# ziqin-h/GIVEPose

Measured on AMD Instinct MI355X. Metric: images/sec PoseNet fwd, bs=64 256x256 fp16, 1/2/4/8 MI355X; % MFMA roofline, higher is better.
Workload: dtype f16

## Files before the change

### givepose_amd/_lib.py

```python
import ctypes
import os
from ctypes import POINTER, Structure, c_char_p, c_double, c_float, c_int, c_long, c_void_p

_HERE = os.path.dirname(os.path.abspath(__file__))
LIB_PATH = os.environ.get("GP_LIB_PATH") or os.path.join(_HERE, "libgivepose_hip.so")

ABI_VERSION = 326
GP_F32, GP_F16, GP_F64 = 0, 1, 2
ACT_NONE, ACT_GELU, ACT_RELU, ACT_LRELU = 0, 1, 2, 3
EPI_NONE, EPI_GELU, EPI_RELU, EPI_LRELU, EPI_SCALE_RES, EPI_RES_RELU, EPI_LNFOLD_GELU = 0, 1, 2, 3, 4, 5, 6
ROT_6D, ROT_6D_Y, ROT_6D_Z, ROT_QUAT, ROT_EULER = 0, 1, 2, 3, 4
KC_GEMM, KC_DCNV3, KC_DWCONV_LN, KC_NORM, KC_ELEMENTWISE, KC_SMALL, KC_COUNT = 0, 1, 2, 3, 4, 5, 6
KC_NAMES = ["gemm", "dcnv3", "dwconv_ln", "norm", "elementwise", "small"]


class GemmDesc(Structure):
    _fields_ = [("X", c_void_p), ("W", c_void_p), ("bias", c_void_p), ("gamma", c_void_p), ("residual", c_void_p),
                ("C", c_void_p), ("workspace", c_void_p),
                ("M", c_int), ("N", c_int), ("K", c_int), ("ldx", c_int), ("ldc", c_int), ("ldres", c_int),
                ("epilogue", c_int), ("out_f32", c_int), ("splitk", c_int),
                ("B", c_int), ("H", c_int), ("Win", c_int), ("Cin", c_int), ("KH", c_int), ("KW", c_int),
                ("stride", c_int), ("pad", c_int), ("Ho", c_int), ("Wo", c_int), ("dtype", c_int),
                ("gn_partial", c_void_p), ("gn_groups", c_int), ("gn_hw", c_int), ("variant", c_int),
                ("ln_stats", c_void_p), ("ln_colsum", c_void_p), ("ln_nslab", c_int), ("ln_eps", c_float),
                ("co_scheduled", c_int), ("prefetch", c_void_p), ("prefetch_bytes", c_long),
                ("split_shift", c_int), ("x_plane_stride", c_long), ("w_plane_stride", c_long),
                ("out_planes", c_int), ("c_plane_stride", c_long),
                ("residual_f32", c_int), ("c16", c_void_p), ("ldc16", c_int), ("gn_rows", c_int)]


# ... 5 lines not shown
    "gp_dcnv3_forward": ([_P, _P, _P, _P] + [c_int] * 9 + [c_float] + [c_int] * 7 + [_P], c_int),
    "gp_dcnv3_forward_any": ([_P] * 4 + [c_int] * 13 + [c_float] + [c_int] * 3 + [_P], c_int),
    "gp_dcnv3_backward": ([_P] * 7 + [c_long, c_long] + [c_int] * 13 + [c_float] + [c_int] * 3 + [_P], c_int),
    "gp_gemm": ([POINTER(GemmDesc), _P], c_int),
    "gp_gemm_gn_rows": ([c_int] * 4, c_int),
    "gp_split_planes": ([_P, _P, c_long, c_int, c_long, c_long, c_int, _P], c_int),
    "gp_convnext_mlp_pack_w2": ([_P, _P, c_int, _P], c_int),
    "gp_convnext_mlp_pack_w2_s32": ([_P, _P, c_int, _P], c_int),
    "gp_convnext_mlp": ([_P] * 8 + [c_long, c_int, c_int, _P], c_int),
    "gp_convnext_stem": ([_P] * 6 + [c_int] * 4 + [c_float, c_int, _P], c_int),
    "gp_dwconv_ln": ([_P] * 6 + [c_int] * 5 + [c_float, c_int, c_long, c_int, _P], c_int),
    "gp_dwconv_ln_groups": ([_P] * 6 + [c_int] * 5 + [c_float, c_int, _P, c_int, _P], c_int),
    "gp_dwconv7_raw_stats": ([_P] * 5 + [c_int] * 5 + [_P], c_int),
    "gp_layernorm": ([_P] * 4 + [c_long, c_int, c_float, c_int, c_int, _P], c_int),
    "gp_groupnorm_chunks": ([c_int, c_int], c_int),
    "gp_groupnorm_stats": ([_P] * 2 + [c_int] * 5 + [_P], c_int),
    "gp_groupnorm_apply": ([_P] * 5 + [c_int] * 4 + [c_float] + [c_int] * 4 + [_P], c_int),
    "gp_groupnorm_upsample2x": ([_P] * 5 + [c_int] * 5 + [c_float] + [c_int] * 3 + [_P], c_int),
    "gp_groupnorm_apply_xyz": ([_P] * 8 + [c_int] * 4 + [c_float] + [c_int] * 3 + [_P], c_int),
    "gp_upsample_bilinear2x": ([_P, _P] + [c_int] * 5 + [_P], c_int),
    "gp_deconv_col2im": ([_P, _P] + [c_int] * 5 + [_P], c_int),
    "gp_xyz_out_layer": ([_P] * 5 + [c_int] * 4 + [_P], c_int),
    "gp_pointwise_k3": ([_P] * 4 + [c_long, c_int, c_int, _P], c_int),
    "gp_pnp_conv1": ([_P] * 4 + [c_int] * 4 + [_P], c_int),
    "gp_xyz_conv3x3_s2": ([_P] * 3 + [c_int] * 4 + [_P], c_int),
    "gp_size_head": ([_P] * 8 + [c_int] * 5 + [_P], c_int),
    "gp_pose_tail": ([_P, _P, c_int] + [_P] * 10 + [c_int, c_int] + [_P] * 5 + [c_int, _P], c_int),
    "gp_pose_tail_rt": ([_P, _P, c_int] + [_P] * 10 + [c_int] * 5 + [_P] * 5 + [c_int, _P], c_int),
    "gp_pnp_conv1_masked": ([_P] * 5 + [c_int] * 4 + [_P], c_int),
    "gp_pool_mmm": ([_P, _P] + [c_int] * 5 + [_P], c_int),
    "gp_patchify_xyz": ([_P, _P, c_int, c_int, c_int, c_int, _P], c_int),
    "gp_attention64": ([_P, _P, c_int, c_int, c_int, _P], c_int),
    "gp_attention64_hd": ([_P, _P] + [c_int] * 4 + [_P], c_int),
    "gp_patchify_pnp": ([_P, _P, _P] + [c_int] * 4 + [_P], c_int),
    "gp_resnet_stem": ([_P] * 4 + [c_int] * 4 + [_P], c_int),
    "gp_maxpool3x3s2": ([_P, _P] + [c_int] * 5 + [_P], c_int),
    "gp_mask_resize_nearest": ([_P, _P, c_int, c_int, c_int, _P], c_int),
    "gp_crop_rois": ([_P] * 12 + [c_int] * 7 + [_P], c_int),
    "gp_pred_rt": ([_P] * 6 + [c_int, _P], c_int),
    "gp_pack_poses": ([_P] * 4 + [c_int, _P], c_int),
    "gp_sn_stem": ([_P] * 4 + [c_int] * 3 + [_P], c_int),
    "gp_sn_pointwise": ([_P] * 6 + [c_long] + [c_int] * 4 + [_P], c_int),
    "gp_sn_depthwise": ([_P] * 4 + [c_int] * 7 + [_P], c_int),
    "gp_sn_avgpool": ([_P] * 2 + [c_int] * 3 + [_P], c_int),
    "gp_sn_se": ([_P] * 6 + [c_int] * 3 + [_P], c_int),
    "gp_sn_head": ([_P] * 12 + [c_int] * 5 + [_P], c_int),
# ... 53 lines not shown
```

### givepose_amd/csrc/dcnv3.hip

```cpp
#include "common.hpp"

namespace {

struct DcnKP {
    const void* in;
    const void* off;
    const void* mask;
    void* out;
    int N, H, W, G, D, K, stride, pad, dil, rc, Ho, Wo, off_ld, mask_ld, logits, xcd;
    float os;
    long rows;
};

template <typename T> struct Ch4;
template <> struct Ch4<half_t> {
    half4 v;
    __device__ __forceinline__ float get(int i) const { return (float)v[i]; }
    __device__ __forceinline__ float fma(float a, int i, float c) const { return fmaf(a, (float)v[i], c); }
    __device__ __forceinline__ float mul(float a, int i) const { return a * (float)v[i]; }
};
template <> struct Ch4<float> {
    f32x4 v;
    __device__ __forceinline__ float get(int i) const { return v[i]; }
    __device__ __forceinline__ float mul(float a, int i) const { return a * v[i]; }
// ... 394 lines not shown

template <typename T, typename OT> int launch(const DcnKP& p, hipStream_t s) {
    if constexpr (sizeof(T) == 2) {
        if (p.G == 4 && p.D == 64 && p.K == 3 && !p.rc && p.Ho % 4 == 0 && p.Wo % 4 == 0 && dcn_patch_enabled() && dcn_wave8_enabled() && !dcn_fold_enabled()) {
            if (dcn_ldsbc_enabled()) hipLaunchKernelGGL((dcnv3_wave8_kernel<OT, true>), dim3(p.N * (p.Ho / 4) * (p.Wo / 4), 2), dim3(256), 0, s, p);
            else hipLaunchKernelGGL((dcnv3_wave8_kernel<OT, false>), dim3(p.N * (p.Ho / 4) * (p.Wo / 4), 2), dim3(256), 0, s, p);
            return 0;
        }
    }
    if (p.G == 4 && p.D == 64 && p.K == 3 && !p.rc && p.Ho % 4 == 0 && p.Wo % 4 == 0 && dcn_patch_enabled()) {
        if (sizeof(T) == 2 && dcn_fold_enabled()) hipLaunchKernelGGL((dcnv3_wave_kernel<T, OT, 3, true, true>), dim3(p.N * (p.Ho / 4) * (p.Wo / 4), 4), dim3(256), 0, s, p);
        else hipLaunchKernelGGL((dcnv3_wave_kernel<T, OT, 3, true>), dim3(p.N * (p.Ho / 4) * (p.Wo / 4), 4), dim3(256), dcn_lds_pad(), s, p);
    } else if (p.G == 4 && p.D == 64 && p.K == 3 && !p.rc) {
        hipLaunchKernelGGL((dcnv3_wave_kernel<T, OT, 3>), dim3(cdiv(p.rows, 4)), dim3(256), 0, s, p);
    } else if (p.G == 4 && p.D == 64 && p.K * p.K - p.rc <= 16) {
        hipLaunchKernelGGL((dcnv3_wave_kernel<T, OT>), dim3(cdiv(p.rows, 4)), dim3(256), 0, s, p);
    } else {
        const long total = p.rows * p.G * (p.D / 4);
        hipLaunchKernelGGL((dcnv3_generic_kernel<T, OT>), dim3(cdiv(total, 256)), dim3(256), 0, s, p);
    }
    return 0;
}

}

extern "C" int gp_dcnv3_forward(const void* in, const void* offset, const void* mask, void* out, int N, int H,
                                int W, int G, int D, int K, int stride, int pad, int dil, float offset_scale,
                                int remove_center, int im2col_step, int off_ld, int mask_ld,
                                int mask_is_logits, int dtype, int om_dtype, void* stream) {
    GP_REQUIRE(in && offset && mask && out, "gp_dcnv3_forward: null pointer");
    GP_REQUIRE(N > 0 && H > 0 && W > 0 && G > 0 && D > 0 && K > 0 && stride > 0 && dil > 0 && pad >= 0,
               "gp_dcnv3_forward: bad geometry");
    GP_REQUIRE(D % 4 == 0, "gp_dcnv3_forward: group_channels=%d must be a multiple of 4", D);
    GP_REQUIRE((dtype == GP_F32 || dtype == GP_F16) && (om_dtype == GP_F32 || om_dtype == GP_F16),
               "gp_dcnv3_forward: bad dtype");
    GP_REQUIRE(!remove_center || (K % 2 == 1), "remove_center is only compatible with odd kernel size.");
    const int step = im2col_step < N ? im2col_step : N;
    GP_REQUIRE(step > 0 && N % step == 0, "batch(%d) must divide im2col_step(%d)", N, step);
    DcnKP p;
    p.in = in; p.off = offset; p.mask = mask; p.out = out;
    p.N = N; p.H = H; p.W = W; p.G = G; p.D = D; p.K = K; p.stride = stride; p.pad = pad; p.dil = dil;
    p.rc = remove_center ? 1 : 0;
    p.Ho = (H + 2 * pad - (dil * (K - 1) + 1)) / stride + 1;
    p.Wo = (W + 2 * pad - (dil * (K - 1) + 1)) / stride + 1;
    GP_REQUIRE(p.Ho > 0 && p.Wo > 0, "gp_dcnv3_forward: empty output");
    const int P = K * K - p.rc;
// ... 16 lines not shown
```

### givepose_amd/csrc/misc.hip

```cpp
#include "common.hpp"

namespace {

__device__ __forceinline__ void store_T(half_t* p, float v) { *p = (half_t)v; }
__device__ __forceinline__ void store_T(float* p, float v) { *p = v; }

template <typename T>
__global__ __launch_bounds__(256) void stem_kernel(const float* __restrict__ img, const float* __restrict__ wt,
                                                   const float* __restrict__ bias, const float* __restrict__ lnw,
                                                   const float* __restrict__ lnb, T* __restrict__ out, int H,
                                                   int W, float eps, int PXB) {
    constexpr int C0 = 128;
    __shared__ __attribute__((aligned(16))) float in_s[12][256];
    const int Ho = H / 4, Wo = W / 4;
    const int tid = threadIdx.x, lane = tid & 63, wave = tid >> 6;
    const int nwb = Wo / PXB;
    const int wblk = blockIdx.x % nwb;
    const int ho = (blockIdx.x / nwb) % Ho;
    const int b = blockIdx.x / (nwb * Ho);
    const int wo0 = wblk * PXB;
    for (int i = tid; i < 12 * PXB * 4; i += 256) {
        const int row = i / (PXB * 4), col = i - row * (PXB * 4);
        const int c = row >> 2, kh = row & 3;
        in_s[row][col] = img[(((long)b * 3 + c) * H + (ho * 4 + kh)) * W + wo0 * 4 + col];
// ... 1037 lines not shown
    GP_REQUIRE(x && w && b && out_nchw && out_nhwc4 && B > 0, "gp_xyz_out_layer: bad argument");
    GP_DT_OK(dtype);
    const int esz = dtype == GP_F16 ? 2 : 4, vec = 16 / esz, chunks = C / vec;
    GP_REQUIRE(C % vec == 0 && (chunks & (chunks - 1)) == 0, "gp_xyz_out_layer: C=%d", C);
    const int LPP = chunks < 64 ? chunks : 64, ppw = 64 / LPP;
    const long rows = (long)B * HW;
    hipStream_t s = (hipStream_t)stream;
    gp_timing_before(s, GP_KC_SMALL, 6.0 * rows * C, (double)rows * C * esz + rows * 28.0);
    dim3 grid(cdiv(rows, 4L * ppw));
    if (dtype == GP_F16) hipLaunchKernelGGL(xyz_out_kernel<half_t>, grid, dim3(256), 0, s, (const half_t*)x, w, b, out_nchw, out_nhwc4, rows, HW, C);
    else hipLaunchKernelGGL(xyz_out_kernel<float>, grid, dim3(256), 0, s, (const float*)x, w, b, out_nchw, out_nhwc4, rows, HW, C);
    GP_LAUNCH_CHECK("gp_xyz_out_layer");
}

extern "C" int gp_pointwise_k3(const float* xyz4, const float* w, const float* b, void* y, long rows, int Cout,
                               int dtype, void* stream) {
    GP_REQUIRE(xyz4 && w && b && y && rows > 0, "gp_pointwise_k3: bad argument");
    GP_DT_OK(dtype);
    const int esz = dtype == GP_F16 ? 2 : 4, vec = 16 / esz;
    GP_REQUIRE(Cout % vec == 0 && 256 % (Cout / vec) == 0, "gp_pointwise_k3: Cout=%d", Cout);
    hipStream_t s = (hipStream_t)stream;
    const long total = cdiv(rows, (256 / (Cout / vec)) * 8) * 256;
    gp_timing_before(s, GP_KC_ELEMENTWISE, 6.0 * rows * Cout, rows * 16.0 + (double)rows * Cout * esz);
    if (dtype == GP_F16) hipLaunchKernelGGL(pointwise_k3_kernel<half_t>, dim3(cdiv(total, 256)), dim3(256), 0, s, xyz4, w, b, (half_t*)y, rows, Cout);
    else hipLaunchKernelGGL(pointwise_k3_kernel<float>, dim3(cdiv(total, 256)), dim3(256), 0, s, xyz4, w, b, (float*)y, rows, Cout);
    GP_LAUNCH_CHECK("gp_pointwise_k3");
}

template <int CIN>
static int launch_smallcin(const float* xyz4, const float* coord2d, const float* w, void* y, int B, int R, int Cout,
                           int dtype, void* stream, const char* name, const float* mask = nullptr) {
    GP_REQUIRE(xyz4 && w && y && B > 0 && R % 8 == 0, "%s: bad argument", name);
    GP_DT_OK(dtype);
    GP_REQUIRE(Cout % 4 == 0 && Cout / 4 <= 256 && 256 % (Cout / 4) == 0, "%s: Cout=%d", name, Cout);
    hipStream_t s = (hipStream_t)stream;
    const long pix = (long)B * (R / 2) * (R / 2);
        const size_t lds = (size_t)CIN * 9 * Cout * sizeof(float);
    gp_timing_before(s, GP_KC_SMALL, 2.0 * pix * CIN * 9 * Cout, (double)B * R * R * CIN * 4 + (double)pix * Cout * (dtype == GP_F16 ? 2 : 4));
    static const bool mfma = [] { const char* e = getenv("GP_SMALLCIN_MFMA"); return !(e && e[0] == '0'); }();
    if (dtype == GP_F16 && mfma && R == 64 && (Cout == 128 || Cout == 256)) {
        if (Cout == 128) hipLaunchKernelGGL((smallcin_conv3x3s2_mfma_kernel<CIN, 2>), dim3(B * (R / 4)), dim3(256), 0, s, xyz4, coord2d, w, (half_t*)y, B, R, mask);
        else hipLaunchKernelGGL((smallcin_conv3x3s2_mfma_kernel<CIN, 4>), dim3(B * (R / 4)), dim3(256), 0, s, xyz4, coord2d, w, (half_t*)y, B, R, mask);
    } else if (dtype == GP_F16)
        hipLaunchKernelGGL((smallcin_conv3x3s2_kernel<half_t, CIN>), dim3(cdiv(pix / 4, 256 / (Cout / 4))), dim3(256), lds, s, xyz4, coord2d, w, (half_t*)y, B, R, Cout, mask);
    else
        hipLaunchKernelGGL((smallcin_conv3x3s2_kernel<float, CIN>), dim3(cdiv(pix / 4, 256 / (Cout / 4))), dim3(256), lds, s, xyz4, coord2d, w, (float*)y, B, R, Cout, mask);
// ... 220 lines not shown
```

### givepose_amd/ops.py

```python
import ctypes
import os

import torch

from . import _lib
from ._lib import (ACT_GELU, ACT_LRELU, ACT_NONE, ACT_RELU, EPI_GELU, EPI_LNFOLD_GELU, EPI_LRELU, EPI_NONE, EPI_RELU, EPI_RES_RELU,
                   EPI_SCALE_RES, GP_F16, GP_F32, GP_F64, GemmDesc, check)

__all__ = ["dtype_code", "gemm", "conv2d_nhwc", "dcnv3_forward", "dcnv3_backward", "dcnv3_forward_into", "convnext_stem", "dwconv_ln",
           "layernorm", "groupnorm", "upsample_bilinear2x", "deconv_col2im", "xyz_out_layer", "pointwise_k3",
           "pnp_conv1", "pnp_conv1_masked", "pool_mmm", "xyz_conv3x3_s2", "size_head", "pose_tail", "pose_tail_rt", "mask_resize_nearest"]


def _L():
    return _lib.load()


def _stream():
    return ctypes.c_void_p(torch.cuda.current_stream().cuda_stream)


def dtype_code(dt):
    if dt == torch.float16:
        return GP_F16
    if dt == torch.float32:
        return GP_F32
    raise TypeError(f"unsupported dtype {dt} (float16 / float32)")


def _ptr(t):
    return None if t is None else ctypes.c_void_p(t.data_ptr())

# ... 421 lines not shown
          "gp_upsample_bilinear2x")
    return out


def deconv_col2im(cols, out, B, H, W_, C):
    code = dtype_code(out.dtype) | (0x400 if cols.dtype == torch.float16 else 0)
    check(_L().gp_deconv_col2im(_ptr(cols), _ptr(out), B, H, W_, C, code, _stream()), "gp_deconv_col2im")
    return out


def xyz_out_layer(x, w, b, out_nchw, out_nhwc4):
    B, HW, C = x.shape
    check(_L().gp_xyz_out_layer(_ptr(_contig(x, "x")), _ptr(w), _ptr(b), _ptr(out_nchw), _ptr(out_nhwc4), B, HW, C,
                                dtype_code(x.dtype), _stream()), "gp_xyz_out_layer")


def pointwise_k3(xyz4, w, b, out):
    rows = xyz4.shape[0]
    check(_L().gp_pointwise_k3(_ptr(xyz4), _ptr(w), _ptr(b), _ptr(out), rows, w.shape[0], dtype_code(out.dtype), _stream()),
          "gp_pointwise_k3")
    return out


def pnp_conv1(xyz4, coord2d, w, out, B, R):
    check(_L().gp_pnp_conv1(_ptr(xyz4), _ptr(_contig(coord2d, "coord2d")), _ptr(w), _ptr(out), B, R, w.shape[1],
                            dtype_code(out.dtype), _stream()), "gp_pnp_conv1")
    return out


def pnp_conv1_masked(xyz4, coord2d, mask, w, out, B, R):
    check(_L().gp_pnp_conv1_masked(_ptr(xyz4), _ptr(_contig(coord2d, "coord2d")), _ptr(_contig(_chk(mask, "mask", torch.float32), "mask")),
                                   _ptr(w), _ptr(out), B, R, w.shape[1], dtype_code(out.dtype), _stream()), "gp_pnp_conv1_masked")
    return out


def pool_mmm(x, out, k):
    B, HW, C = x.shape
    if x.dtype != out.dtype or tuple(out.shape) != (B, k * C):
        raise ValueError(f"pool_mmm: out {tuple(out.shape)} {out.dtype} for x {tuple(x.shape)} {x.dtype}, k={k}")
    check(_L().gp_pool_mmm(_ptr(_contig(x, "x")), _ptr(_contig(out, "out")), B, HW, C, k, dtype_code(x.dtype), _stream()), "gp_pool_mmm")
    return out


def xyz_conv3x3_s2(xyz4, w, out, B, R):
    check(_L().gp_xyz_conv3x3_s2(_ptr(xyz4), _ptr(w), _ptr(out), B, R, w.shape[1], dtype_code(out.dtype), _stream()),
          "gp_xyz_conv3x3_s2")
# ... 47 lines not shown
```

### givepose_amd/posenet.py

```python
import ctypes
import os
from collections import OrderedDict

import numpy as np
import torch
import torch.nn as nn

from . import _lib, ops, synth
from ._lib import (ACT_GELU, ACT_RELU, EPI_GELU, EPI_LNFOLD_GELU, EPI_LRELU, EPI_NONE, EPI_SCALE_RES)
from .config import FLAT_OPS, ROT_TYPES, PoseNetConfig, validate

OM_LD = 128


class _Node(nn.Module):
    """Container mirroring one level of the reference module tree (names only)."""


def _register(root, name, tensor, is_param):
    parts = name.split(".")
    mod = root
    for p in parts[:-1]:
        if p not in mod._modules:
            mod.add_module(p, _Node())
        mod = mod._modules[p]
    if is_param:
        mod.register_parameter(parts[-1], tensor)
    else:
        mod.register_buffer(parts[-1], tensor)


FUSE_GN_UPSAMPLE = os.environ.get("GP_FUSE_GN_UPSAMPLE", "1") != "0"

_BUFFER_SUFFIXES = ("running_mean", "running_var", "num_batches_tracked")

# ... 145 lines not shown
                W[q + "qkv_w"] = gw(a(f"block.{i}.attn.qkv.weight"))
                W[q + "proj_w"], W[q + "proj_b"] = gw(a(f"block.{i}.attn.proj.weight")), f32(a(f"block.{i}.attn.proj.bias"))
                W[q + "fc1_w"], W[q + "fc1_b"] = gw(a(f"block.{i}.mlp.fc1.weight")), f32(a(f"block.{i}.mlp.fc1.bias"))
                W[q + "fc2_w"], W[q + "fc2_b"] = gw(a(f"block.{i}.mlp.fc2.weight")), f32(a(f"block.{i}.mlp.fc2.bias"))
        for li, i in enumerate((0, 3, 6) if cfg.nocsmap_encoder == "conv" else ()):
            p, q = f"nocs_encoder.features.{i}.", f"enc{li}."
            if cfg.use_dcn == "dcnv3":
                cw = sd[p + "conv.weight"].reshape(256, -1)
                W[q + "conv_w"] = f32(cw) if li == 0 else gw(cw)
                W[q + "conv_b"] = f32(sd[p + "conv.bias"])
                d = p + "dcnv3."
                W[q + "dw_w"] = lowp(sd[d + "dw_conv.0.weight"].reshape(256, 9).t())
                W[q + "dw_b"] = f32(sd[d + "dw_conv.0.bias"])
                W[q + "ln_w"], W[q + "ln_b"] = f32(sd[d + "dw_conv.1.1.weight"]), f32(sd[d + "dw_conv.1.1.bias"])
                omw = torch.cat([sd[d + "offset.weight"], sd[d + "mask.weight"]], 0)
                omb = torch.cat([sd[d + "offset.bias"], sd[d + "mask.bias"]], 0)
                W[q + "om_w"] = gw(torch.cat([omw, omw.new_zeros(OM_LD - omw.shape[0], omw.shape[1])], 0))
                W[q + "om_b"] = f32(torch.cat([omb, omb.new_zeros(OM_LD - omb.shape[0])], 0))
                W[q + "in_w"], W[q + "in_b"] = gw(sd[d + "input_proj.weight"]), f32(sd[d + "input_proj.bias"])
                wf = sd[d + "input_proj.weight"] @ cw
                W[q + "fold_w"] = f32(wf) if li == 0 else gw(wf)
                W[q + "fold_b"] = f32(sd[d + "input_proj.weight"] @ sd[p + "conv.bias"] + sd[d + "input_proj.bias"])
                W[q + "out_w"], W[q + "out_b"] = gw(sd[d + "output_proj.weight"]), f32(sd[d + "output_proj.bias"])
            else:
                cw = sd[p + "weight"]
                W[q + "conv_w"] = f32(cw.reshape(256, -1).t()) if li == 0 else gw(cw.permute(0, 2, 3, 1).reshape(256, -1))
            W[q + "gn_w"], W[q + "gn_b"] = f32(sd[f"nocs_encoder.features.{i + 1}.weight"]), f32(sd[f"nocs_encoder.features.{i + 1}.bias"])
        W["red.w"], W["red.b"] = gw(sd["feat_reducer.weight"].reshape(256, -1)), f32(sd["feat_reducer.bias"])
        if cfg.pnp_head == "att":
            a = lambda k: sd["pnp_net." + k]
            W["apn.pe_w"] = gw(a("patch_embed.proj.weight").permute(0, 2, 3, 1).reshape(192, -1))
            W["apn.pe_b"] = f32(a("patch_embed.proj.bias"))
            W["apn.pos"] = f32(a("pos_embed").reshape(64, 192))
            W["apn.ones"] = torch.ones(192, dtype=torch.float32, device=device)
            W["apn.norm_w"], W["apn.norm_b"] = f32(a("norm.weight")), f32(a("norm.bias"))
            for i in range(3):
                q = f"apn{i}."
                for n in ("norm1", "norm2"):
                    W[q + n + "_w"], W[q + n + "_b"] = f32(a(f"block.{i}.{n}.weight")), f32(a(f"block.{i}.{n}.bias"))
                W[q + "qkv_w"] = gw(a(f"block.{i}.attn.qkv.weight"))
                W[q + "proj_w"], W[q + "proj_b"] = gw(a(f"block.{i}.attn.proj.weight")), f32(a(f"block.{i}.attn.proj.bias"))
                W[q + "fc1_w"], W[q + "fc1_b"] = gw(a(f"block.{i}.mlp.fc1.weight")), f32(a(f"block.{i}.mlp.fc1.bias"))
                W[q + "fc2_w"], W[q + "fc2_b"] = gw(a(f"block.{i}.mlp.fc2.weight")), f32(a(f"block.{i}.mlp.fc2.bias"))
        else:
            W["pnp.c0_w"] = f32(sd["pnp_net.features.0.weight"].reshape(128, -1).t())
            for li, i in enumerate((0, 3, 6)):
# ... 53 lines not shown
                h = S // (2 << li)
                for n in ("a", "b", "c"):
                    buf[f"rs{li}{n}"] = e(B, h, h, planes)
        for s, d in enumerate(dims):
            h = H >> s
            if cfg.res_fp32 and T == torch.float16 and d == 512:
                buf[f"x{s}"], buf[f"x{s}h"] = f(B, h, h, d), e(B, h, h, d)
            else:
                buf[f"x{s}"] = e(B, h, h, d)
            buf[f"t{s}"] = e(B, h, h, d)
            buf[f"h{s}"] = e(B * h * h, 4 * d)
            if d == 512:
                buf["ln_stats"] = f(B * h * h, 2, d // 128)
            if s > 0:
                buf[f"dsn{s}"] = e(B, h * 2, h * 2, dims[s - 1])
        buf["cols"] = e(B * 64, 9 * 256) if (T == torch.float16 and cfg.deconv_cols_f16 and os.environ.get("GP_DECONV_COLS_F32") != "1") else f(B * 64, 9 * 256)
        for r in (16, 32, 64):
            buf[f"ya{r}"], buf[f"yb{r}"] = e(B, r, r, 256), e(B, r, r, 256)
        chunks = max(ops.groupnorm_chunks(B, r * r) for r in (8, 16, 32, 64))
        buf["gn_partial"], buf["size_scratch"] = f(B * max(chunks, R * R // 16) * 32 * 2), f(B * (cfg.feat_ts + (512 if cfg.main_backbone == "resnet34" else cfg.convnext_dims[-1])))
        buf["nocs_nchw"], buf["nocs_nhwc4"] = f(B, 3, R, R), f(B * R * R, 4)
        buf["ivfc_nchw"], buf["ivfc_nhwc4"] = f(B, 3, R, R), f(B * R * R, 4)
        buf["mask_out"], buf["size"] = f(B, 1, R, R), f(B, 3)
        for li, r in enumerate((64, 32, 16)):
            buf[f"e_in{li}"], buf[f"e_proj{li}"] = e(B, r, r, 256), e(B, r, r, 256)
            buf[f"e_x1{li}"] = e(B * r * r // 4, 256)
            buf[f"e_om{li}"] = f(B * r * r // 4, OM_LD)
            buf[f"e_g{li}"], buf[f"e_o{li}"] = e(B, r // 2, r // 2, 256), e(B, r // 2, r // 2, 256)
        if cfg.nocsmap_encoder == "att":
            buf["a_patch"], buf["a_x"], buf["a_h"] = e(B * 64, 192), e(B * 64, 256), e(B * 64, 256)
            buf["a_qkv"], buf["a_att"], buf["a_mlp"] = e(B * 64, 768), e(B * 64, 256), e(B * 64, 1024)
            buf["a_pos"] = self._packed["att.pos"].to(T).repeat(B, 1).contiguous()
        buf["feat_cat"] = e(B, 8, 8, 512)
        if cfg.pnp_head == "att":
            buf["p_patch"], buf["p_x"], buf["p_h"] = e(B * 64, 320), e(B * 64, 192), e(B * 64, 192)
            buf["p_qkv"], buf["p_att"], buf["p_mlp"], buf["p_flat"] = e(B * 64, 576), e(B * 64, 192), e(B * 64, 768), e(B * 64, 192)
            buf["p_pos"] = self._packed["apn.pos"].to(T).repeat(B, 1).contiguous()
        else:
            buf["p0"], buf["p1"], buf["p2"] = e(B, 32, 32, 128), e(B, 16, 16, 128), e(B, 8, 8, 128)
        buf["fc1"] = e(B, 2048)
        buf["hh"], buf["hz"] = f(B, 256), f(B, 256)
        if FLAT_OPS[cfg.flat_op]:
            buf["pooled"] = e(B, 128 * FLAT_OPS[cfg.flat_op])
        buf["pred_rot"], buf["pred_t"], buf["rot_allo"], buf["rot_ego"], buf["trans"] = f(B, cfg.rot_dim), f(B, 3), f(B, 9), f(B, 9), f(B, 3)
        buf["rot6d"] = buf["pred_rot"] if cfg.rot_dim == 6 else None
        plan = {"buf": buf, "graph": None, "warm": False, "ragged": bool(ragged)}
        if ragged:
            buf["grp"] = torch.arange(B, dtype=torch.int32, device=device)
            buf["grp_host"] = torch.arange(B, dtype=torch.int32).pin_memory()
            for k in ("roi_img", "roi_mask", "roi_coord_2d", "bbox_center", "mean_size"):
                buf[k].zero_()
            buf["roi_wh"].fill_(1.0)
            buf["resize_ratio"].fill_(1.0)
            buf["cam_K"].copy_(torch.eye(3, device=device).expand(B, 3, 3))
        self._plans[key] = plan
        self._evict_plans(key)
        return plan

    def _gn(self, x, w, b, act, buf, G=32, out=None, ldy=None, fused=False, out_planes=False, rows=64):
        B = x.shape[0]
        C = x.shape[-1]
        xv = x.view(B, -1, C)
        ops.groupnorm(xv, w, b, xv if out is None else out, G, act, buf["gn_partial"], ldy=ldy, fused_stats=fused, out_planes=out_planes, rows=rows)

    def _gnrows(self, M, N, K, hw):
        if self.split_gemm or self.compute_dtype != torch.float16 or os.environ.get("GP_GN_ROWS64") == "1":
            return 64
        return ops.gemm_gn_rows(M, N, K, hw)

# ... 126 lines not shown
            ops.gemm(buf["a_patch"], W["att.pe_w"], x, bias=W["att.pe_b"], epilogue=EPI_SCALE_RES, gamma=W["att.ones"],
                     residual=buf["a_pos"])
            for i in range(3):
                q = f"att{i}."
                h = ops.layernorm(x, W[q + "norm1_w"], W[q + "norm1_b"], buf["a_h"], eps=1e-5)
                ops.gemm(h, W[q + "qkv_w"], buf["a_qkv"])
                ops.attention64(buf["a_qkv"], buf["a_att"], B, 8)
                ops.gemm(buf["a_att"], W[q + "proj_w"], x, bias=W[q + "proj_b"], epilogue=EPI_SCALE_RES, gamma=W["att.ones"], residual=x)
                h = ops.layernorm(x, W[q + "norm2_w"], W[q + "norm2_b"], buf["a_h"], eps=1e-5)
                ops.gemm(h, W[q + "fc1_w"], buf["a_mlp"], bias=W[q + "fc1_b"], epilogue=EPI_GELU)
                ops.gemm(buf["a_mlp"], W[q + "fc2_w"], x, bias=W[q + "fc2_b"], epilogue=EPI_SCALE_RES, gamma=W["att.ones"], residual=x)
            ops.layernorm(x, W["att.norm_w"], W["att.norm_b"], cat2d[:, 256:], eps=1e-5, ldy=512)
        for li, r in enumerate((64, 32, 16) if cfg.nocsmap_encoder == "conv" else ()):
            q = f"enc{li}."
            ro = r // 2
            if only_layer is not None:
                if li != only_layer:
                    continue
                prev = buf[f"e_o{li - 1}"]
                if weights_of is not None:
                    q = f"enc{weights_of}."
            if cfg.use_dcn == "dcnv3":
                xin = buf[f"e_in{li}"]
                if li == 0:
                    ops.pointwise_k3(buf["nocs_nhwc4"], W[q + "fold_w"], W[q + "fold_b"], buf[f"e_proj{li}"].view(-1, 256))
                else:
                    ops.gemm(prev.view(-1, 256), W[q + "fold_w"], buf[f"e_proj{li}"].view(-1, 256), bias=W[q + "fold_b"])
                if plan.get("ragged"):
                    if li == 0:
                        ops.pointwise_k3(buf["nocs_nhwc4"], W[q + "conv_w"], W[q + "conv_b"], xin.view(-1, 256))
                    else:
                        ops.gemm(prev.view(-1, 256), W[q + "conv_w"], xin.view(-1, 256), bias=W[q + "conv_b"])
                    ops.dwconv_ln_groups(xin, W[q + "dw_w"], W[q + "dw_b"], W[q + "ln_w"], W[q + "ln_b"], buf[f"e_x1{li}"], 3, buf["grp"], act=ACT_GELU)
                    ops.gemm(buf[f"e_x1{li}"], W[q + "om_w"], buf[f"e_om{li}"], bias=W[q + "om_b"])
                    ops.dcnv3_forward_into(buf[f"e_proj{li}"], buf[f"e_om{li}"], buf[f"e_om{li}"][:, 72:], buf[f"e_g{li}"], 3, 2, 1, 1, 4, 64, 1.0,
                                           off_ld=OM_LD, mask_ld=OM_LD, mask_is_logits=True)
                Bg = self.dcn_couple if (self.dcn_couple and B > self.dcn_couple) else B
                if plan.get("ragged"):
                    Bg = B + 1
                if B % Bg and not plan.get("ragged"):
                    raise ValueError(f"batch {B} is not a multiple of dcn_couple = {Bg}")
                for g0 in range(0, B if not plan.get("ragged") else 0, Bg):
                    gs = slice(g0, g0 + Bg)
                    nq = Bg * ro * ro
                    npre = min(Bg * r * r, (nq + r + 8 + 15) // 16 * 16)
                    xin_g = xin[gs]
                    if li == 0:
                        ops.pointwise_k3(buf["nocs_nhwc4"][g0 * r * r:][:npre], W[q + "conv_w"], W[q + "conv_b"], xin_g.view(-1, 256)[:npre])
                    else:
                        ops.gemm(prev[gs].view(-1, 256)[:npre], W[q + "conv_w"], xin_g.view(-1, 256)[:npre], bias=W[q + "conv_b"])
                    x1_g = buf[f"e_x1{li}"][g0 * r * r // 4:(g0 + Bg) * r * r // 4]
                    om_g = buf[f"e_om{li}"][g0 * r * r // 4:(g0 + Bg) * r * r // 4]
                    ops.dwconv_ln(xin_g, W[q + "dw_w"], W[q + "dw_b"], W[q + "ln_w"], W[q + "ln_b"], x1_g, 3, act=ACT_GELU, n_pixels=nq)
                    ops.gemm(x1_g, W[q + "om_w"], om_g, bias=W[q + "om_b"])
                    ops.dcnv3_forward_into(buf[f"e_proj{li}"][gs], om_g, om_g[:, 72:], buf[f"e_g{li}"][gs], 3, 2, 1, 1, 4, 64, 1.0,
                                           off_ld=OM_LD, mask_ld=OM_LD, mask_is_logits=True)
                y = buf[f"e_o{li}"]
                ops.gemm(buf[f"e_g{li}"].view(-1, 256), W[q + "out_w"], y.view(-1, 256), bias=W[q + "out_b"],
                         gn=self._gnarg(buf, ro * ro))
                fused = True
                if only_layer is not None:
                    return
            else:
                y = buf[f"e_o{li}"]
                fused = li > 0
                if li == 0:
                    ops.xyz_conv3x3_s2(buf["nocs_nhwc4"], W[q + "conv_w"], y, B, r)
                else:
                    ops.conv2d_nhwc(prev, W[q + "conv_w"], 3, 3, 2, 1, out=y, gn=self._gnarg(buf, ro * ro))
            if li < 2:
                self._gn(y, W[q + "gn_w"], W[q + "gn_b"], ACT_RELU, buf, fused=fused)
                prev = y
            else:
                self._gn(y, W[q + "gn_w"], W[q + "gn_b"], ACT_RELU, buf, out=cat2d[:, 256:], ldy=512, fused=fused)

    def _seq_pnp(self, B, plan):
        W, buf, cfg = self._packed, plan["buf"], self.cfg
        R = cfg.out_res
        k = FLAT_OPS[cfg.flat_op]
        if cfg.pnp_head == "att":
# ... 206 lines not shown
```

### include/givepose_hip.h

```cpp
#ifndef GIVEPOSE_HIP_H
#define GIVEPOSE_HIP_H

#ifdef __cplusplus
extern "C" {
#endif

enum gp_status { GP_OK = 0, GP_ERR_INVALID = -1, GP_ERR_LAUNCH = -2, GP_ERR_RUNTIME = -3 };
enum gp_dtype { GP_F32 = 0, GP_F16 = 1, GP_F64 = 2  };
#define GP_OUT_PLANES 0x100
#define GP_IN_F32 0x200
#define GP_SPLIT_SHIFT 11
enum gp_act { GP_ACT_NONE = 0, GP_ACT_GELU = 1, GP_ACT_RELU = 2, GP_ACT_LRELU = 3  };
enum gp_epilogue {
    GP_EPI_NONE = 0,
    GP_EPI_GELU = 1,
    GP_EPI_RELU = 2,
    GP_EPI_LRELU = 3,
    GP_EPI_SCALE_RES = 4,
    GP_EPI_RES_RELU = 5,
    GP_EPI_LNFOLD_GELU = 6
};

const char* gp_last_error(void);
#define GP_ABI_VERSION 326
int gp_version(void);
int gp_device_info(int* cu_count, char* arch, int arch_len);

int gp_dcnv3_forward(const void* in, const void* offset, const void* mask, void* out, int N, int H, int W,
                     int G, int D, int K, int stride, int pad, int dil, float offset_scale,
                     int remove_center, int im2col_step, int off_ld, int mask_ld, int mask_is_logits,
                     int dtype, int om_dtype, void* stream);

int gp_dcnv3_forward_any(const void* in, const void* offset, const void* mask, void* out, int N, int H, int W, int G,
                         int D, int kernel_h, int kernel_w, int stride_h, int stride_w, int pad_h, int pad_w,
                         int dilation_h, int dilation_w, float offset_scale, int remove_center, int im2col_step,
                         int dtype, void* stream);

int gp_dcnv3_backward(const void* in, const void* offset, const void* mask, const void* grad_out, void* grad_in,
                      void* grad_offset, void* grad_mask, long offset_numel, long mask_numel, int N, int H, int W, int G,
                      int D, int kernel_h, int kernel_w, int stride_h, int stride_w, int pad_h, int pad_w,
                      int dilation_h, int dilation_w, float offset_scale, int remove_center, int im2col_step,
                      int dtype, void* stream);

typedef struct gp_gemm_desc {
    const void* X;
    const void* W;
    const float* bias;
// ... 60 lines not shown
int gp_groupnorm_apply(const void* x, const float* partial, const float* w, const float* b, void* y, int B,
                       int HW, int C, int G, float eps, int act, int ldy, int chunks ,
                       int dtype, void* stream);

int gp_groupnorm_upsample2x(const void* x, const float* partial, const float* w, const float* b, void* y, int B, int H, int W,
                            int C, int G, float eps, int act, int chunks, int dtype, void* stream);

#define GP_ACT_PACKED16 0x100
int gp_groupnorm_apply_xyz(const void* x, const float* partial, const float* w, const float* b, const float* out_w,
                           const float* out_b, float* out_nchw, float* out_nhwc4, int B, int HW, int C, int G,
                           float eps, int act, int chunks, int dtype, void* stream);

int gp_upsample_bilinear2x(const void* x, void* y, int B, int H, int W, int C, int dtype, void* stream);

#define GP_COLS_F16 0x400
int gp_deconv_col2im(const void* cols, void* out, int B, int H, int W, int C, int dtype, void* stream);

int gp_xyz_out_layer(const void* x, const float* w, const float* b, float* out_nchw, float* out_nhwc4,
                     int B, int HW, int C, int dtype, void* stream);

int gp_pointwise_k3(const float* xyz4, const float* w, const float* b, void* y, long rows, int Cout,
                    int dtype, void* stream);

int gp_pnp_conv1(const float* xyz4, const float* coord2d, const float* w, void* y, int B, int R, int Cout,
                 int dtype, void* stream);

int gp_pnp_conv1_masked(const float* xyz4, const float* coord2d, const float* mask, const float* w, void* y, int B, int R,
                        int Cout, int dtype, void* stream);

int gp_pool_mmm(const void* x, void* out, int B, int HW, int C, int k, int dtype, void* stream);

int gp_xyz_conv3x3_s2(const float* xyz4, const float* w, void* y, int B, int R, int Cout, int dtype,
                      void* stream);

int gp_size_head(const void* feat, const float* w1, const float* b1, const float* w2, const float* b2,
                 const float* mean_size, float* size, float* scratch, int B, int HW, int C, int F, int dtype,
                 void* stream);

int gp_pose_tail(const float* h, const float* hz, int ldh, const float* w_r, const float* b_r,
                 const float* w_t, const float* b_t, const float* w_z, const float* b_z, const float* cam_K,
                 const float* bbox_center, const float* resize_ratio, const float* roi_wh, int wild6d,
                 int site_centroid, float* rot6d, float* pred_t, float* rot_allo, float* rot_ego,
                 float* trans, int B, void* stream);

enum gp_rot_kind { GP_ROT_6D = 0, GP_ROT_6D_Y = 1, GP_ROT_6D_Z = 2, GP_ROT_QUAT = 3, GP_ROT_EULER = 4 };

// ... 71 lines not shown
```

Baseline: 12410.

## Fold encoder layer-0 DCNv3 into a 3-channel xyz sampling and 16x256 projection

The first encoder layer is linear from the 3-channel NOCS map up to the DCNv3 sampling. Its 1x1 conv, input_proj and output_proj are therefore folded algebraically on the host (in float64) into one 256x16 matrix plus a bias. A new fused kernel bilinearly samples the 4-channel xyz map from LDS for each of the 4 groups and 9 taps, then applies the folded projection. It writes fp16 output together with GroupNorm partial statistics, removing the 256-channel pointwise projection, the full 256-channel deformable sampling and the output GEMM along with their intermediate buffers. It is hard-wired to 64x64, K3 stride 2 geometry and fp16 non-split mode, and changes rounding because the arithmetic stays in fp32 rather than going through fp16 intermediates.

```diff
diff --git a/givepose_amd/_lib.py b/givepose_amd/_lib.py
--- a/givepose_amd/_lib.py
+++ b/givepose_amd/_lib.py
@@ -5,7 +5,7 @@
 _HERE = os.path.dirname(os.path.abspath(__file__))
 LIB_PATH = os.environ.get("GP_LIB_PATH") or os.path.join(_HERE, "libgivepose_hip.so")
 
-ABI_VERSION = 326
+ABI_VERSION = 327
 GP_F32, GP_F16, GP_F64 = 0, 1, 2
 ACT_NONE, ACT_GELU, ACT_RELU, ACT_LRELU = 0, 1, 2, 3
 EPI_NONE, EPI_GELU, EPI_RELU, EPI_LRELU, EPI_SCALE_RES, EPI_RES_RELU, EPI_LNFOLD_GELU = 0, 1, 2, 3, 4, 5, 6
@@ -57,6 +57,7 @@
     "gp_deconv_col2im": ([_P, _P] + [c_int] * 5 + [_P], c_int),
     "gp_xyz_out_layer": ([_P] * 5 + [c_int] * 4 + [_P], c_int),
     "gp_pointwise_k3": ([_P] * 4 + [c_long, c_int, c_int, _P], c_int),
+    "gp_dcnv3_xyz_project": ([_P] * 6 + [c_long] + [c_int] * 14 + [_P], c_int),
     "gp_pnp_conv1": ([_P] * 4 + [c_int] * 4 + [_P], c_int),
     "gp_xyz_conv3x3_s2": ([_P] * 3 + [c_int] * 4 + [_P], c_int),
     "gp_size_head": ([_P] * 8 + [c_int] * 5 + [_P], c_int),
diff --git a/givepose_amd/csrc/dcnv3.hip b/givepose_amd/csrc/dcnv3.hip
--- a/givepose_amd/csrc/dcnv3.hip
+++ b/givepose_amd/csrc/dcnv3.hip
@@ -440,6 +440,171 @@
     return 0;
 }
 
+struct XyzKP {
+    const f32x4* xyz;
+    const float* om;
+    const float* m;
+    const float* bias;
+    void* out;
+    float* gn;
+    long rows;
+    int om_ld, mask_col, logits;
+};
+
+template <typename T, int WAVES>
+__global__ __launch_bounds__(WAVES * 64) void dcnv3_xyz_project_kernel(const XyzKP p) {
+    constexpr int NT = WAVES * 64, PX = WAVES * 32, H = 64, W = 64, U = 4;
+    __shared__ __attribute__((aligned(16))) f32x4 map_s[H * W];
+    __shared__ __attribute__((aligned(16))) f32x4 v_s[PX * 4];
+    const int lane = threadIdx.x & 63, t = lane & 15, g = lane >> 4;
+    const int wave = __builtin_amdgcn_readfirstlane(threadIdx.x >> 6);
+    const long pb = (long)blockIdx.x * PX;
+    const int crop = (int)(pb >> 10);
+    const long r0 = pb + wave * 32;
+    const bool live = r0 < p.rows;
+    {
+        const f32x4* src = p.xyz + (long)crop * (H * W);
+#pragma unroll 8
+        for (int i = 0; i < H * W / NT; ++i) map_s[i * NT + threadIdx.x] = src[i * NT + threadIdx.x];
+    }
+    const bool own = t < 9 && live;
+    const float* omp = p.om + r0 * p.om_ld + (g * 9 + t) * 2;
+    const float* mkp = p.om + r0 * p.om_ld + p.mask_col + g * 9 + t;
+    f32x2 o_n[U];
+    float m_n[U];
+    auto fetch = [&](int it0) {
+#pragma unroll
+        for (int u = 0; u < U; ++u) {
+            o_n[u] = f32x2{0.f, 0.f};
+            m_n[u] = p.logits ? -INFINITY : 0.f;
+            if (own) {
+                o_n[u] = *reinterpret_cast<const f32x2*>(omp + (long)(it0 + u) * p.om_ld);
+                m_n[u] = mkp[(long)(it0 + u) * p.om_ld];
+            }
+        }
+    };
+    fetch(0);
+    __syncthreads();
+    const int ti = t / 3, tj = t - ti * 3;
+    const float os = 1.f, Hf = (float)H, Wf = (float)W;
+#pragma unroll 1
+    for (int it0 = 0; it0 < 32; it0 += U) {
+        f32x2 o_c[U];
+        float m_c[U];
+#pragma unroll
+        for (int u = 0; u < U; ++u) { o_c[u] = o_n[u]; m_c[u] = m_n[u]; }
+        if (it0 + U < 32) fetch(it0 + U);
+#pragma unroll
+        for (int u = 0; u < U; ++u) {
+            const int pl = (int)(r0 & 1023) + it0 + u;
+            const int ho = pl >> 5, wo = pl & 31;
+            const float ow = o_c[u][0], oh = o_c[u][1];
+            float m = m_c[u];
+            if (p.logits) {
+                const float mx = group_max(m, 16);
+                const float e = t < 9 ? expf(m - mx) : 0.f;
+                const float sm = group_sum(e, 16);
+                m = e / sm;
+            }
+            const float p0_w_ = (float)(1 - 1 + wo * 2) - 1 * os;
+            const float p0_h_ = (float)(1 - 1 + ho * 2) - 1 * os;
+            float loc_w = p0_w_ + (ti * 1 + ow) * os;
+            float loc_h = p0_h_ + (tj * 1 + oh) * os;
+            const bool in = t < 9 && loc_h > -1.f && loc_w > -1.f && loc_h < Hf && loc_w < Wf;
+            loc_w = in ? loc_w : 0.f;
+            loc_h = in ? loc_h : 0.f;
+            m = in ? m : 0.f;
+            const float fh = floorf(loc_h), fw = floorf(loc_w);
+            const float lh = loc_h - fh, lw = loc_w - fw, hh = 1.f - lh, hw = 1.f - lw;
+            const int h_low = (int)fh, w_low = (int)fw, h_high = h_low + 1, w_high = w_low + 1;
+            const bool hl = h_low >= 0, hhi = h_high <= H - 1, wl = w_low >= 0, whi = w_high <= W - 1;
+            const float w1 = (hl && wl) ? hh * hw : 0.f, w2 = (hl && whi) ? hh * lw : 0.f;
+            const float w3 = (hhi && wl) ? lh * hw : 0.f, w4 = (hhi && whi) ? lh * lw : 0.f;
+            const int y0 = max(h_low, 0), y1 = min(h_high, H - 1), x0 = max(w_low, 0), x1 = min(w_high, W - 1);
+            const f32x4 v1 = map_s[y0 * W + x0], v2 = map_s[y0 * W + x1], v3 = map_s[y1 * W + x0], v4 = map_s[y1 * W + x1];
+            f32x4 s;
+#pragma unroll
+            for (int c = 0; c < 3; ++c) {
+                float tt = w1 * v1[c];
+                tt = fmaf(w2, v2[c], tt);
+                tt = fmaf(w3, v3[c], tt);
+                tt = fmaf(w4, v4[c], tt);
+                s[c] = group_sum(tt * m, 16);
+            }
+            s[3] = group_sum((((w1 + w2) + w3) + w4) * m, 16);
+            if (t == 0) v_s[(wave * 32 + it0 + u) * 4 + g] = s;
+        }
+    }
+    __syncthreads();
+    if (!live) return;
+    f32x4 mr[4][4];
+#pragma unroll
+    for (int c = 0; c < 4; ++c)
+#pragma unroll
+        for (int k = 0; k < 4; ++k) mr[c][k] = *reinterpret_cast<const f32x4*>(p.m + (lane * 4 + c) * 16 + k * 4);
+    const f32x4 b4 = *reinterpret_cast<const f32x4*>(p.bias + lane * 4);
+    float gs = 0.f, gq = 0.f;
+    T* op = reinterpret_cast<T*>(p.out) + r0 * 256 + lane * 4;
+#pragma unroll 2
+    for (int px = 0; px < 32; ++px) {
+        const f32x4* vp = v_s + (wave * 32 + px) * 4;
+        f32x4 a[4];
+#pragma unroll
+        for (int k = 0; k < 4; ++k) a[k] = vp[k];
+        float acc[4];
+#pragma unroll
+        for (int c = 0; c < 4; ++c) {
+            float x = b4[c];
+#pragma unroll
+            for (int k = 0; k < 4; ++k)
+#pragma unroll
+                for (int j = 0; j < 4; ++j) x = fmaf(mr[c][k][j], a[k][j], x);
+            acc[c] = x;
+        }
+        gs += (acc[0] + acc[1]) + (acc[2] + acc[3]);
+        gq += (acc[0] * acc[0] + acc[1] * acc[1]) + (acc[2] * acc[2] + acc[3] * acc[3]);
+        st4(op + (long)px * 256, acc);
+    }
+    gs = group_sum(gs, 2);
+    gq = group_sum(gq, 2);
+    if ((lane & 1) == 0)
+        *reinterpret_cast<f32x2*>(p.gn + ((r0 >> 5) * 32 + (lane >> 1)) * 2) = f32x2{gs, gq};
+}
+
+}
+
+extern "C" int gp_dcnv3_xyz_project(const float* xyz4, const float* om, const float* m, const float* bias, void* out, float* gn_partial,
+                                    long rows, int H, int W, int K, int stride, int pad, int dil, int G, int om_ld, int mask_col,
+                                    int mask_is_logits, int gn_groups, int gn_hw, int gn_rows, int dtype, void* stream) {
+    GP_REQUIRE(xyz4 && om && m && bias && out && gn_partial, "gp_dcnv3_xyz_project: null pointer");
+    GP_REQUIRE(H == 64 && W == 64 && K == 3 && stride == 2 && pad == 1 && dil == 1 && G == 4,
+               "gp_dcnv3_xyz_project: geometry %dx%d K%d s%d p%d d%d G%d is not the encoder's (64x64 K3 s2 p1 d1 G4)", H, W, K, stride, pad, dil, G);
+    GP_REQUIRE(rows > 0 && rows % 32 == 0, "gp_dcnv3_xyz_project: rows=%ld must be a positive multiple of 32", rows);
+    GP_REQUIRE(dtype == GP_F32 || dtype == GP_F16, "gp_dcnv3_xyz_project: bad dtype");
+    GP_REQUIRE(mask_col >= 72 && om_ld >= mask_col + 36 && om_ld % 2 == 0, "gp_dcnv3_xyz_project: om_ld=%d mask_col=%d", om_ld, mask_col);
+    GP_REQUIRE(gn_groups == 32 && gn_hw == 1024 && gn_rows == 32, "gp_dcnv3_xyz_project: GroupNorm statistics come per 32 rows of 32 groups of a 32x32 map (gn_groups=%d gn_hw=%d gn_rows=%d)",
+               gn_groups, gn_hw, gn_rows);
+    GP_REQUIRE(((uintptr_t)xyz4 | (uintptr_t)out | (uintptr_t)m | (uintptr_t)bias) % 16 == 0 && ((uintptr_t)om | (uintptr_t)gn_partial) % 8 == 0,
+               "gp_dcnv3_xyz_project: misaligned pointer");
+    XyzKP p;
+    p.xyz = reinterpret_cast<const f32x4*>(xyz4); p.om = om; p.m = m; p.bias = bias; p.out = out; p.gn = gn_partial;
+    p.rows = rows; p.om_ld = om_ld; p.mask_col = mask_col; p.logits = mask_is_logits ? 1 : 0;
+    hipStream_t s = (hipStream_t)stream;
+    const int esz = dtype == GP_F16 ? 2 : 4;
+    const double crops = (double)((rows + 1023) / 1024);
+    gp_timing_before(s, GP_KC_DCNV3, (double)rows * (36 * 4 * 4 * 2.0 + 256 * 16 * 2.0), crops * H * W * 16 + (double)rows * 108 * 4 + (double)rows * 256 * esz);
+    gp_timing_label("dcnv3_xyz_project rows%ld", rows);
+    const bool big = rows >= 32 * 1024;
+    const long grid = (rows + (big ? 256 : 64) - 1) / (big ? 256 : 64);
+    GP_REQUIRE(grid < (1l << 31), "gp_dcnv3_xyz_project: grid too large");
+    if (dtype == GP_F16) {
+        if (big) hipLaunchKernelGGL((dcnv3_xyz_project_kernel<half_t, 8>), dim3((unsigned)grid), dim3(512), 0, s, p);
+        else hipLaunchKernelGGL((dcnv3_xyz_project_kernel<half_t, 2>), dim3((unsigned)grid), dim3(128), 0, s, p);
+    } else {
+        if (big) hipLaunchKernelGGL((dcnv3_xyz_project_kernel<float, 8>), dim3((unsigned)grid), dim3(512), 0, s, p);
+        else hipLaunchKernelGGL((dcnv3_xyz_project_kernel<float, 2>), dim3((unsigned)grid), dim3(128), 0, s, p);
+    }
+    GP_LAUNCH_CHECK("gp_dcnv3_xyz_project");
 }
 
 extern "C" int gp_dcnv3_forward(const void* in, const void* offset, const void* mask, void* out, int N, int H,
diff --git a/givepose_amd/csrc/misc.hip b/givepose_amd/csrc/misc.hip
--- a/givepose_amd/csrc/misc.hip
+++ b/givepose_amd/csrc/misc.hip
@@ -1083,6 +1083,7 @@
     hipStream_t s = (hipStream_t)stream;
     const long total = cdiv(rows, (256 / (Cout / vec)) * 8) * 256;
     gp_timing_before(s, GP_KC_ELEMENTWISE, 6.0 * rows * Cout, rows * 16.0 + (double)rows * Cout * esz);
+    gp_timing_label("pointwise_k3 rows%ld Cout%d", rows, Cout);
     if (dtype == GP_F16) hipLaunchKernelGGL(pointwise_k3_kernel<half_t>, dim3(cdiv(total, 256)), dim3(256), 0, s, xyz4, w, b, (half_t*)y, rows, Cout);
     else hipLaunchKernelGGL(pointwise_k3_kernel<float>, dim3(cdiv(total, 256)), dim3(256), 0, s, xyz4, w, b, (float*)y, rows, Cout);
     GP_LAUNCH_CHECK("gp_pointwise_k3");
diff --git a/givepose_amd/ops.py b/givepose_amd/ops.py
--- a/givepose_amd/ops.py
+++ b/givepose_amd/ops.py
@@ -7,7 +7,7 @@
 from ._lib import (ACT_GELU, ACT_LRELU, ACT_NONE, ACT_RELU, EPI_GELU, EPI_LNFOLD_GELU, EPI_LRELU, EPI_NONE, EPI_RELU, EPI_RES_RELU,
                    EPI_SCALE_RES, GP_F16, GP_F32, GP_F64, GemmDesc, check)
 
-__all__ = ["dtype_code", "gemm", "conv2d_nhwc", "dcnv3_forward", "dcnv3_backward", "dcnv3_forward_into", "convnext_stem", "dwconv_ln",
+__all__ = ["dtype_code", "gemm", "conv2d_nhwc", "dcnv3_forward", "dcnv3_backward", "dcnv3_forward_into", "dcnv3_xyz_project", "convnext_stem", "dwconv_ln",
            "layernorm", "groupnorm", "upsample_bilinear2x", "deconv_col2im", "xyz_out_layer", "pointwise_k3",
            "pnp_conv1", "pnp_conv1_masked", "pool_mmm", "xyz_conv3x3_s2", "size_head", "pose_tail", "pose_tail_rt", "mask_resize_nearest"]
 
@@ -475,6 +475,21 @@
     return out
 
 
+def dcnv3_xyz_project(xyz4, om, m, bias, out, gn, mask_col=72, mask_is_logits=True):
+    _contig(_chk(xyz4, "xyz4"), "xyz4"), _contig(_chk(om, "om"), "om"), _contig(_chk(out, "out"), "out")
+    rows = out.shape[0]
+    if xyz4.dtype != torch.float32 or om.dtype != torch.float32 or m.dtype != torch.float32 or bias.dtype != torch.float32:
+        raise TypeError("dcnv3_xyz_project: xyz4, om, m and bias are float32")
+    if tuple(m.shape) != (256, 16) or bias.numel() != 256 or out.shape[1] != 256 or om.shape[0] < rows or xyz4.shape[0] < (rows + 1023) // 1024 * 4096:
+        raise RuntimeError("dcnv3_xyz_project: shapes")
+    if gn[0].numel() < (rows + 1023) // 1024 * 32 * 32 * 2:
+        raise RuntimeError("dcnv3_xyz_project: the gn_partial buffer is too small for 32 chunks of 32 groups per crop")
+    check(_L().gp_dcnv3_xyz_project(_ptr(xyz4), _ptr(om), _ptr(_contig(m, "m")), _ptr(bias), _ptr(out), _ptr(gn[0]), rows, 64, 64, 3, 2, 1, 1, 4,
+                                    om.shape[1], mask_col, 1 if mask_is_logits else 0, gn[1], gn[2], gn[3], dtype_code(out.dtype), _stream()),
+          "gp_dcnv3_xyz_project")
+    return out
+
+
 def pnp_conv1(xyz4, coord2d, w, out, B, R):
     check(_L().gp_pnp_conv1(_ptr(xyz4), _ptr(_contig(coord2d, "coord2d")), _ptr(w), _ptr(out), B, R, w.shape[1],
                             dtype_code(out.dtype), _stream()), "gp_pnp_conv1")
diff --git a/givepose_amd/posenet.py b/givepose_amd/posenet.py
--- a/givepose_amd/posenet.py
+++ b/givepose_amd/posenet.py
@@ -11,6 +11,16 @@
 from .config import FLAT_OPS, ROT_TYPES, PoseNetConfig, validate
 
 OM_LD = 128
+
+
+def enc0_xyz_pack(sd, prefix="nocs_encoder.features.0.", dtype=torch.float32):
+    f64 = lambda k: sd[prefix + k].detach().to(device="cpu", dtype=torch.float64)
+    cw, cb = f64("conv.weight").reshape(256, -1), f64("conv.bias")
+    iw, ib = f64("dcnv3.input_proj.weight"), f64("dcnv3.input_proj.bias")
+    ow, ob = f64("dcnv3.output_proj.weight"), f64("dcnv3.output_proj.bias")
+    fold = torch.cat([iw @ cw, (iw @ cb + ib)[:, None]], 1)
+    m = torch.cat([ow[:, 64 * g:64 * g + 64] @ fold[64 * g:64 * g + 64] for g in range(4)], 1)
+    return m.to(dtype).contiguous(), ob.to(dtype).contiguous()
 
 
 class _Node(nn.Module):
@@ -202,6 +212,8 @@
                 W[q + "fold_w"] = f32(wf) if li == 0 else gw(wf)
                 W[q + "fold_b"] = f32(sd[d + "input_proj.weight"] @ sd[p + "conv.bias"] + sd[d + "input_proj.bias"])
                 W[q + "out_w"], W[q + "out_b"] = gw(sd[d + "output_proj.weight"]), f32(sd[d + "output_proj.bias"])
+                if li == 0 and T == torch.float16 and not self.split_gemm:
+                    W[q + "xyz_m"], W[q + "xyz_b"] = (f32(t) for t in enc0_xyz_pack(sd, p))
             else:
                 cw = sd[p + "weight"]
                 W[q + "conv_w"] = f32(cw.reshape(256, -1).t()) if li == 0 else gw(cw.permute(0, 2, 3, 1).reshape(256, -1))
@@ -301,11 +313,13 @@
         buf["nocs_nchw"], buf["nocs_nhwc4"] = f(B, 3, R, R), f(B * R * R, 4)
         buf["ivfc_nchw"], buf["ivfc_nhwc4"] = f(B, 3, R, R), f(B * R * R, 4)
         buf["mask_out"], buf["size"] = f(B, 1, R, R), f(B, 3)
+        enc0_xyz = "enc0.xyz_m" in self._packed and os.environ.get("GP_ENC0_XYZ") != "0"
         for li, r in enumerate((64, 32, 16)):
-            buf[f"e_in{li}"], buf[f"e_proj{li}"] = e(B, r, r, 256), e(B, r, r, 256)
-            buf[f"e_x1{li}"] = e(B * r * r // 4, 256)
+            buf[f"e_in{li}"], buf[f"e_x1{li}"] = e(B, r, r, 256), e(B * r * r // 4, 256)
             buf[f"e_om{li}"] = f(B * r * r // 4, OM_LD)
-            buf[f"e_g{li}"], buf[f"e_o{li}"] = e(B, r // 2, r // 2, 256), e(B, r // 2, r // 2, 256)
+            buf[f"e_o{li}"] = e(B, r // 2, r // 2, 256)
+            if li > 0 or not enc0_xyz:
+                buf[f"e_proj{li}"], buf[f"e_g{li}"] = e(B, r, r, 256), e(B, r // 2, r // 2, 256)
         if cfg.nocsmap_encoder == "att":
             buf["a_patch"], buf["a_x"], buf["a_h"] = e(B * 64, 192), e(B * 64, 256), e(B * 64, 256)
             buf["a_qkv"], buf["a_att"], buf["a_mlp"] = e(B * 64, 768), e(B * 64, 256), e(B * 64, 1024)
@@ -323,7 +337,7 @@
             buf["pooled"] = e(B, 128 * FLAT_OPS[cfg.flat_op])
         buf["pred_rot"], buf["pred_t"], buf["rot_allo"], buf["rot_ego"], buf["trans"] = f(B, cfg.rot_dim), f(B, 3), f(B, 9), f(B, 9), f(B, 3)
         buf["rot6d"] = buf["pred_rot"] if cfg.rot_dim == 6 else None
-        plan = {"buf": buf, "graph": None, "warm": False, "ragged": bool(ragged)}
+        plan = {"buf": buf, "graph": None, "warm": False, "ragged": bool(ragged), "enc0_xyz": enc0_xyz}
         if ragged:
             buf["grp"] = torch.arange(B, dtype=torch.int32, device=device)
             buf["grp_host"] = torch.arange(B, dtype=torch.int32).pin_memory()
@@ -496,7 +510,12 @@
                     q = f"enc{weights_of}."
             if cfg.use_dcn == "dcnv3":
                 xin = buf[f"e_in{li}"]
-                if li == 0:
+                xyz0 = li == 0 and plan.get("enc0_xyz") and only_layer is None
+                if xyz0:
+                    nb = B if (plan.get("ragged") or not (self.dcn_couple and B > self.dcn_couple)) else self.dcn_couple
+                    if nb % min(nb, 256):
+                        raise RuntimeError(f"gp_dcnv3_forward: batch({nb}) must divide im2col_step({min(nb, 256)})")
+                elif li == 0:
                     ops.pointwise_k3(buf["nocs_nhwc4"], W[q + "fold_w"], W[q + "fold_b"], buf[f"e_proj{li}"].view(-1, 256))
                 else:
                     ops.gemm(prev.view(-1, 256), W[q + "fold_w"], buf[f"e_proj{li}"].view(-1, 256), bias=W[q + "fold_b"])
@@ -507,8 +526,9 @@
                         ops.gemm(prev.view(-1, 256), W[q + "conv_w"], xin.view(-1, 256), bias=W[q + "conv_b"])
                     ops.dwconv_ln_groups(xin, W[q + "dw_w"], W[q + "dw_b"], W[q + "ln_w"], W[q + "ln_b"], buf[f"e_x1{li}"], 3, buf["grp"], act=ACT_GELU)
                     ops.gemm(buf[f"e_x1{li}"], W[q + "om_w"], buf[f"e_om{li}"], bias=W[q + "om_b"])
-                    ops.dcnv3_forward_into(buf[f"e_proj{li}"], buf[f"e_om{li}"], buf[f"e_om{li}"][:, 72:], buf[f"e_g{li}"], 3, 2, 1, 1, 4, 64, 1.0,
-                                           off_ld=OM_LD, mask_ld=OM_LD, mask_is_logits=True)
+                    if not xyz0:
+                        ops.dcnv3_forward_into(buf[f"e_proj{li}"], buf[f"e_om{li}"], buf[f"e_om{li}"][:, 72:], buf[f"e_g{li}"], 3, 2, 1, 1, 4, 64, 1.0,
+                                               off_ld=OM_LD, mask_ld=OM_LD, mask_is_logits=True)
                 Bg = self.dcn_couple if (self.dcn_couple and B > self.dcn_couple) else B
                 if plan.get("ragged"):
                     Bg = B + 1
@@ -527,9 +547,16 @@
                     om_g = buf[f"e_om{li}"][g0 * r * r // 4:(g0 + Bg) * r * r // 4]
                     ops.dwconv_ln(xin_g, W[q + "dw_w"], W[q + "dw_b"], W[q + "ln_w"], W[q + "ln_b"], x1_g, 3, act=ACT_GELU, n_pixels=nq)
                     ops.gemm(x1_g, W[q + "om_w"], om_g, bias=W[q + "om_b"])
-                    ops.dcnv3_forward_into(buf[f"e_proj{li}"][gs], om_g, om_g[:, 72:], buf[f"e_g{li}"][gs], 3, 2, 1, 1, 4, 64, 1.0,
-                                           off_ld=OM_LD, mask_ld=OM_LD, mask_is_logits=True)
+                    if not xyz0:
+                        ops.dcnv3_forward_into(buf[f"e_proj{li}"][gs], om_g, om_g[:, 72:], buf[f"e_g{li}"][gs], 3, 2, 1, 1, 4, 64, 1.0,
+                                               off_ld=OM_LD, mask_ld=OM_LD, mask_is_logits=True)
                 y = buf[f"e_o{li}"]
+                if xyz0:
+                    ops.dcnv3_xyz_project(buf["nocs_nhwc4"], buf["e_om0"], W[q + "xyz_m"], W[q + "xyz_b"], y.view(-1, 256),
+                                          gn=self._gnarg(buf, ro * ro, 32))
+                    self._gn(y, W[q + "gn_w"], W[q + "gn_b"], ACT_RELU, buf, fused=True, rows=32)
+                    prev = y
+                    continue
                 ops.gemm(buf[f"e_g{li}"].view(-1, 256), W[q + "out_w"], y.view(-1, 256), bias=W[q + "out_b"],
                          gn=self._gnarg(buf, ro * ro))
                 fused = True
diff --git a/include/givepose_hip.h b/include/givepose_hip.h
--- a/include/givepose_hip.h
+++ b/include/givepose_hip.h
@@ -22,7 +22,7 @@
 };
 
 const char* gp_last_error(void);
-#define GP_ABI_VERSION 326
+#define GP_ABI_VERSION 327
 int gp_version(void);
 int gp_device_info(int* cu_count, char* arch, int arch_len);
 
@@ -129,6 +129,10 @@
 int gp_pointwise_k3(const float* xyz4, const float* w, const float* b, void* y, long rows, int Cout,
                     int dtype, void* stream);
 
+int gp_dcnv3_xyz_project(const float* xyz4, const float* om, const float* m, const float* bias, void* out, float* gn_partial,
+                         long rows, int H, int W, int K, int stride, int pad, int dil, int G, int om_ld, int mask_col,
+                         int mask_is_logits, int gn_groups, int gn_hw, int gn_rows, int dtype, void* stream);
+
 int gp_pnp_conv1(const float* xyz4, const float* coord2d, const float* w, void* y, int B, int R, int Cout,
                  int dtype, void* stream);
 
```

Result: faster. 12620, median of 6 (+1.7%).
